# THUDM/GCC

Hardware: AMD Instinct MI355X
Metric: sampled-subgraphs/sec (higher is better)
Workload: dtype f32

## Files before the change

### gcc_amd/csrc/posemb.hip

```cpp
#include <mutex>
#include "host_common.h"
#include <type_traits>

namespace {

constexpr int kJMax = GCC_POSEMB_LDS_MAX;
#ifndef GCC_POSEMB_SMALL_T
#define GCC_POSEMB_SMALL_T 256
#endif
constexpr int kSmallT = GCC_POSEMB_SMALL_T;
constexpr int kJSmall = 64;

constexpr int kMaxViews = GCC_POSEMB_MAX_VIEWS;
struct PosView {
    const int32_t *node_off, *row_ptr, *col_idx;
    float *pos, *evals, *raw;
};
struct PosMulti {
    PosView v[kMaxViews];
    int32_t nviews, B, hidden;
    uint64_t seed;
    int32_t *status;
    long long *ticks;
};
// ... 2090 lines not shown
                }
                __syncthreads();
                orth(j + 1, -1);
                float s3 = 0.f;
                for (int r = tid; r < n; r += kKThreads) s3 = fmaf(w[r], w[r], s3);
                nrm = sqrtf(block_sum(s3, red));
                beta = 0.f;
            } else {
                nrm = beta;
            }
            if (tid == 0) H[(j + 1) * kM + j] = beta;
            for (int r = tid; r < n; r += kKThreads) {
                const float vn = w[r] / nrm;
                V[(int64_t)(j + 1) * ldv + r] = vn;
                x[r] = vn * dinv[r];
            }
            __syncthreads();
        }
        PHASE_TICK(0);
        for (int i = tid; i < kM * lda; i += kKThreads) {
            const int r = i / lda, c = i - r * lda;
            float v = 0.f;
            if (c < kM) v = r <= c ? H[r * kM + c] : H[c * kM + r];
            Aj[i] = v;
        }
        __syncthreads();
        tridiagonalize<1, kKThreads, 2>(Aj, lda, kM, tw);
        eig_top_values<kKThreads, kVecCap>(tw, kM, keep, es);
        const bool ritz_failed = eig_top_vectors<1, kKThreads>(Aj, lda, kM, keep, tw, es,
                                                               (uint32_t)a.seed ^ ((uint32_t)gb * 0x9E3779B1u) ^ (uint32_t)cycle,
                                                               nullptr, tick_);
        PHASE_TICK(1);
        if (tid < kM) {
            theta[tid] = tid < keep ? es.lamv[tid] : -2.f;
            sel[tid] = tid < keep ? tid : kM;
        }
        if (tid == 0) { done = 1; flag = ritz_failed ? 2 : 0; }
        __syncthreads();
        const float beta_m = H[kM * kM + (kM - 1)];
        if (tid < k) {
            const float res = fabsf(beta_m * Yj[(kM - 1) * lda + tid]);
            if (res > kRitzTol) done = 0;
            if (res > 10.f * kRitzTol) flag = 2;
        }
        __syncthreads();
        const bool finished = done != 0 || cycle == kMaxCycles - 1;
#ifdef GCC_AMD_HIPEMU
        if (getenv("GCC_POSEMB_DEBUG") && tid == 0) {
            float worst = 0.f; int nbad = 0;
            for (int i = 0; i < kM; ++i) if (sel[i] < k) { const float rs = fabsf(beta_m * Yj[(kM - 1) * lda + i]); worst = rs > worst ? rs : worst; nbad += rs > kRitzTol; }
            fprintf(stderr, "kry b=%d n=%d cycle=%d worst=%.2e nbad=%d theta_k=%.4f\n", b, n, cycle + 1, worst, nbad, 0.f);
        }
#endif
        if (finished && done == 0 && flag == 2 && tid == 0) {
            atomicOr(a.status, (int32_t)GCC_STATUS_POSEMB_NOT_CONVERGED);
            if (atomicAdd(a.status + 4, 1) == 0) { a.status[5] = gb; a.status[6] = kClsKrylov; a.status[7] = n; a.status[8] = -1; a.status[9] = n; }
        }
        if (finished && done == 0 && tid == 0) atomicAdd(a.status + 3, 1);
        const int nout = finished ? k : keep;
        if (tid < kM) {
            const int t = finished ? k - 1 - sel[tid] : sel[tid];
            if (t >= 0 && t < nout) colsrc[t] = tid;
        }
        __syncthreads();
        if (!finished) {
            const int nchunk = (nout + 7) >> 3;
            for (int task = tid; task < n * nchunk; task += kKThreads) {
                const int ch = task / n, r = task - ch * n;
                float acc[8] = {0.f, 0.f, 0.f, 0.f, 0.f, 0.f, 0.f, 0.f};
                int src[8];
#pragma unroll
                for (int u = 0; u < 8; ++u) src[u] = colsrc[min(8 * ch + u, nout - 1)];
                for (int c = 0; c < kM; ++c) {
                    const float v = V[(int64_t)c * ldv + r];
#pragma unroll
                    for (int u = 0; u < 8; ++u) acc[u] = fmaf(v, Yj[c * lda + src[u]], acc[u]);
                }
#pragma unroll
                for (int u = 0; u < 8; ++u)
                    if (8 * ch + u < nout) Valt[(int64_t)(8 * ch + u) * ldv + r] = acc[u];
            }
            for (int r = tid; r < n; r += kKThreads) Valt[(int64_t)keep * ldv + r] = V[(int64_t)kM * ldv + r];
            for (int i = tid; i < (kM + 1) * kM; i += kKThreads) H[i] = 0.f;
            __syncthreads();
            if (tid < kM && sel[tid] < keep) H[sel[tid] * kM + sel[tid]] = theta[tid];
            __syncthreads();
            float *tmp = V; V = Valt; Valt = tmp;
            j = keep;
            PHASE_TICK(2);
            continue;
        }
        float *rawout = a.raw ? a.raw : a.pos;
        const int nchunk = (k + 7) >> 3;
        for (int task = tid; task < n * nchunk; task += kKThreads) {
            const int ch = task / n, r = task - ch * n;
            float acc[8] = {0.f, 0.f, 0.f, 0.f, 0.f, 0.f, 0.f, 0.f};
            int src[8];
#pragma unroll
            for (int u = 0; u < 8; ++u) src[u] = colsrc[min(8 * ch + u, k - 1)];
            for (int c = 0; c < kM; ++c) {
                const float v = V[(int64_t)c * ldv + r];
#pragma unroll
                for (int u = 0; u < 8; ++u) acc[u] = fmaf(v, Yj[c * lda + src[u]], acc[u]);
            }
            float *ro = rawout + (int64_t)(n0 + r) * a.hidden + 8 * ch;
#pragma unroll
            for (int u = 0; u < 8; ++u)
                if (8 * ch + u < k) ro[u] = acc[u];
        }
        __syncthreads();
        for (int r = tid; r < n; r += kKThreads) {
            const float *ro = rawout + (int64_t)(n0 + r) * a.hidden;
            float *po = a.pos + (int64_t)(n0 + r) * a.hidden;
            float s2 = 0.f;
            for (int c = 0; c < k; ++c) s2 = fmaf(ro[c], ro[c], s2);
            const float inv = s2 > 0.f ? 1.0f / sqrtf(s2) : 1.0f;
            for (int c = 0; c < a.hidden; ++c) {
                const float v = c < k ? ro[c] : 0.f;
                po[c] = v * inv;
                if (a.raw) a.raw[(int64_t)(n0 + r) * a.hidden + c] = v;
            }
        }
        if (a.evals && tid < kM && sel[tid] < k) a.evals[(int64_t)b * a.hidden + (k - 1 - sel[tid])] = theta[tid];
        if (a.evals) for (int c = k + tid; c < a.hidden; c += kKThreads) a.evals[(int64_t)b * a.hidden + c] = 0.f;
        break;
    }
    PHASE_TICK(3);
    if (tid == 0) {
        atomicMax(a.status + 1, cycle + 1);
        atomicAdd(a.status + 2, steps);
    }
    }
}


constexpr int kChP = 64;
constexpr int kChPWide = 64, kChPNarrow = 32;
#ifndef GCC_POSEMB_CH_NARROW_WANT
#define GCC_POSEMB_CH_NARROW_WANT 20
#endif
constexpr int kChNarrowWant = GCC_POSEMB_CH_NARROW_WANT;
constexpr int kChNarrowGuards = 8;
#ifndef GCC_POSEMB_CH_THREADS
#define GCC_POSEMB_CH_THREADS 1024
#endif
constexpr int kChThreads = GCC_POSEMB_CH_THREADS;
static_assert(kChThreads % 64 == 0 && kNodeMax % kChThreads == 0 && kChThreads >= 256 && kChThreads <= 1024, "block-class workgroup size");
constexpr int kChRowsPerThread = kNodeMax / kChThreads;
#if defined(GCC_AMD_HIPEMU) || GCC_POSEMB_CH_THREADS > 512
#define GCC_CHEB_REG_CAP
#else
#define GCC_CHEB_REG_CAP __attribute__((amdgpu_waves_per_eu(GCC_POSEMB_CH_THREADS / 256 + 1)))
#endif
constexpr int kChCsrCap = 12288;
#ifndef GCC_POSEMB_CH_LONGDEG
#define GCC_POSEMB_CH_LONGDEG 32
#endif
constexpr int kChLongDeg = GCC_POSEMB_CH_LONGDEG;
constexpr int kChSlabFloats = 4096;
constexpr int kChMaxChunks = kChSlabFloats / 32;
constexpr int kChMaxLong = kChMaxChunks / 2;
constexpr int kChRounds = 16;
constexpr int kChMaxRitz = 5;
constexpr float kChTol = 2e-5f;
constexpr double kChShift = 1e-8;
constexpr float kChAmpLog = 12.9f;
constexpr int kChBw = 32;

struct LdsYes { static constexpr bool value = true; };
struct LdsNo { static constexpr bool value = false; };

constexpr int64_t kChBufFloats = (int64_t)kNodeMax * kChP;
struct ChebArgs {
    PosMulti m;
    PosHead hd;
    float *xws;
    uint32_t *tabs;
};

template <int P>
struct ChebRitzLds {
    static constexpr int Ldy = P + 1;
    static constexpr int Lf = 0;
    static constexpr int Af = Lf + P * Ldy;
    static constexpr int Y = Af + P * Ldy;
    static constexpr int tri = Y + P * Ldy;
    static constexpr int lu = tri + tri_head_floats(P, P * Ldy, kChThreads);
    static constexpr int bytes = (int)sizeof(float) * lu + tri_lu_bytes(P, kChBw);
};
template <int P>
struct ChebDenseLds {
    static constexpr int G = 0, K = G + P * P, Li = K + P * P;
    static constexpr int bytes = (Li + P * P) * (int)sizeof(double);
};
struct ChebLds {
    static constexpr int crow = 0;
    static constexpr int ccol = crow + (int)sizeof(uint16_t) * (kNodeMax + 8);
    static constexpr int scale = ccol + (int)sizeof(uint16_t) * kChCsrCap;
    static constexpr int slab = scale + (int)sizeof(float) * kNodeMax;
    static constexpr int region = slab + (int)sizeof(float) * kChSlabFloats;
    static constexpr int dense_bytes = ChebDenseLds<kChP>::bytes;
    static constexpr int ritz_pad = kChP * (int)sizeof(float);
    static constexpr int ritz_bytes = ChebRitzLds<kChP>::bytes + ritz_pad;
    static constexpr int region_bytes = ritz_bytes > dense_bytes ? ritz_bytes : dense_bytes;
    static constexpr int bytes = region + region_bytes;
    static_assert(region_bytes >= kNodeMax * kDeflNodeBytes, "the deflation tables overlay the region of the dense matrices");
};

__global__ __launch_bounds__(kChThreads) GCC_CHEB_REG_CAP void posemb_cheb_kernel(ChebArgs ca)
{
    DYN_SMEM(smem);
    __shared__ EigShared es;
    __shared__ float theta[kChP], resid[kChP], dsc[kChP];
    __shared__ double dscd[kChP];
    __shared__ int longrow[kChMaxLong], longfirst[kChMaxLong + 1];
    __shared__ int chunk_beg[kChMaxChunks + 1];
    __shared__ uint8_t chunk_row[kChMaxChunks], rowx[kNodeMax];
    __shared__ int sh_clen, sh_long_t;
    __shared__ int wsum[kChThreads / 64 + 1];
    __shared__ int sh_item, sh_tot[3], sh_nlong, sh_nchunk, sh_fail;
    __shared__ int colsrc[64];
    constexpr int kCls = kClsCheb;
    const PosMulti &m = ca.m;
    const PosHead &hd = ca.hd;
    constexpr int kNW = kChThreads / 64;
    uint16_t *crow = (uint16_t *)(smem + ChebLds::crow);
    uint16_t *ccol = (uint16_t *)(smem + ChebLds::ccol);
    float *scale = (float *)(smem + ChebLds::scale);
    float *slab = (float *)(smem + ChebLds::slab);
    unsigned char *region = smem + ChebLds::region;
    for (;;) {
    __syncthreads();
    if (threadIdx.x == 0) sh_item = atomicAdd(hd.next + kCls, 1);
    __syncthreads();
    if (sh_item >= hd.count[kCls]) return;
    uint32_t tid_ = threadIdx.x;
    opaque_u32(tid_);
    const int tid = (int)tid_, lane = tid & 63, wv = tid >> 6;
    const int gb = hd.list[(int64_t)kCls * hd.T + sh_item] & kItemMask;
    PosArgs a;
    int b;
    item_args(m, gb, a, b);
    const int n0 = a.node_off[b], n = a.node_off[b + 1] - n0;
#ifdef GCC_POSEMB_ABLATE_CHEB
    continue;
#endif
    const int k = min(min(n - 2, a.hidden), kMaxVec);
    long long tick_ = m.ticks ? device_ticks() : 0;
    if (m.ticks && tid == 0) atomicAdd((unsigned long long *)&m.ticks[kCls * 16 + 15], 1ull);
    const int32_t *rp = a.row_ptr + n0;
    float *XA0 = ca.xws + (int64_t)blockIdx.x * 3 * kChBufFloats, *XB0 = XA0 + kChBufFloats, *XC0 = XB0 + kChBufFloats;

    Defl d;
    defl_bind(d, region, kNodeMax);
    for (int i = tid; i < n; i += kChThreads) defl_init_node(d, i, rp, a.col_idx, n0);
    if (tid == 0) { sh_fail = 0; sh_nlong = 0; sh_nchunk = 0; }
    __syncthreads();
    for (int i = tid; i < n; i += kChThreads) defl_count_node(d, i, rp, a.col_idx, n0, hd.use_stalks != 0);
    __syncthreads();
    for (int p = tid; p < n; p += kChThreads) defl_order_node(d, p, rp, a.col_idx, n0);
    __syncthreads();
    defl_prefix_block<kChThreads>(d, n, sh_tot, (int *)slab);
    const int nr = sh_tot[0], z = sh_tot[1], zp = sh_tot[2];
    for (int i = tid; i < n; i += kChThreads) {
        if (d.ridx[i] == kNone) continue;
        const int di = rp[i + 1] - rp[i];
        const int pi = d.par[i];
        float sc = 1.0f / sqrtf((float)(di < 1 ? 1 : di));
        if (pi != (int)kNone && d.tcnt[pi] >= 2) {
            sc = sqrtf((float)d.tcnt[pi]);
        } else {
            const int h = d.phub[pi != (int)kNone ? pi : i];
            if (h != (int)kNone && d.pcnt[h] >= 2) sc = pi != (int)kNone ? 1.0f / sqrtf((float)d.pcnt[h]) : sqrtf(0.5f * (float)d.pcnt[h]);
        }
        scale[d.ridx[i]] = sc;
    }
    for (int r = tid; r <= nr; r += kChThreads) crow[r] = 0;
    __syncthreads();
    for (int i = wv; i < n; i += kNW) {
        if (d.ridx[i] == kNone) continue;
        int c = 0;
        for (int e0 = rp[i]; e0 < rp[i + 1]; e0 += 64) {
            const int e = e0 + lane;
            const bool keep = e < rp[i + 1] && d.ridx[a.col_idx[e] - n0] != kNone;
            c += __popcll(wave_ballot(keep));
        }
        if (lane == 0) crow[d.ridx[i] + 1] = (uint16_t)(c > 65535 ? 65535 : c);
    }
    __syncthreads();
    {
        const int r0 = kChRowsPerThread * tid;
        int c[kChRowsPerThread], own = 0;
#pragma unroll
        for (int u = 0; u < kChRowsPerThread; ++u) { c[u] = r0 + u < nr ? (int)crow[r0 + u + 1] : 0; own += c[u]; }
        int incl = wave_scan_incl(own);
        if (lane == 63) wsum[wv] = incl;
        __syncthreads();
        int base = 0;
        for (int q = 0; q < wv; ++q) base += wsum[q];
        incl += base - own;
        __syncthreads();
#pragma unroll
        for (int u = 0; u < kChRowsPerThread; ++u) {
            incl += c[u];
            if (r0 + u < nr) {
                if (incl > kChCsrCap) sh_fail = 1;
                crow[r0 + u + 1] = (uint16_t)(incl > 65535 ? 65535 : incl);
            }
        }
    }
    __syncthreads();
    if (!sh_fail) {
        for (int i = wv; i < n; i += kNW) {
            if (d.ridx[i] == kNone) continue;
            int at = (int)crow[d.ridx[i]];
            for (int e0 = rp[i]; e0 < rp[i + 1]; e0 += 64) {
                const int e = e0 + lane;
                const int rj = e < rp[i + 1] ? (int)d.ridx[a.col_idx[e] - n0] : (int)kNone;
                const unsigned long long mk = wave_ballot(rj != (int)kNone);
                if (rj != (int)kNone) ccol[at + __popcll(mk & lanemask_lt())] = (uint16_t)rj;
                at += __popcll(mk);
            }
        }
    }
    __syncthreads();
    uint16_t *xrec = (uint16_t *)(ca.tabs + (int64_t)blockIdx.x * kTabFloats);
    for (int v = tid; v < n; v += kChThreads) defl_record(d, v, rp, a.col_idx, n0, xrec + 4 * v);
    __syncthreads();
    PHASE_TICK(0);
    bool failed = sh_fail != 0;
    auto build_chunks = [&](int slots) {
        constexpr int R = kChRowsPerThread;
        const int r0 = R * tid;
        int len[R];
#pragma unroll
        for (int u = 0; u < R; ++u) len[u] = (r0 + u < nr && !failed) ? (int)crow[r0 + u + 1] - (int)crow[r0 + u] : 0;
        auto block_scan = [&](int v, int &total) -> int {
            int incl = wave_scan_incl(v);
            if (lane == 63) wsum[wv] = incl;
            __syncthreads();
            int base = 0, tot = 0;
            for (int q = 0; q < kNW; ++q) { if (q < wv) base += wsum[q]; tot += wsum[q]; }
            __syncthreads();
            total = tot;
            return incl - v + base;
        };
        int T = kChLongDeg, nl = 0, x = 0;
        for (;;) {
            int own = 0;
#pragma unroll
            for (int u = 0; u < R; ++u) own += len[u] > T ? 1 : 0;
            x = block_scan(own, nl);
            if (nl <= slots / 2) break;
            T *= 2;
        }
        int own = 0, total = 0;
#pragma unroll
        for (int u = 0; u < R; ++u) own += len[u] > T ? len[u] : 0;
        (void)block_scan(own, total);
        int clen = nl ? (total + (slots - nl) - 1) / (slots - nl) : 8;
        clen = clen < 8 ? 8 : (clen + 3) & ~3;
        own = 0;
#pragma unroll
        for (int u = 0; u < R; ++u) own += len[u] > T ? (len[u] + clen - 1) / clen : 0;
        int nc = 0;
        int fx = block_scan(own, nc);
#pragma unroll
        for (int u = 0; u < R; ++u) {
            const int r = r0 + u;
            const bool lg = len[u] > T;
            if (r < nr) rowx[r] = lg ? (uint8_t)x : (uint8_t)0xFF;
            if (lg) {
                const int nch = (len[u] + clen - 1) / clen;
                longrow[x] = r;
                longfirst[x] = fx;
                for (int j = 0; j < nch; ++j) { chunk_beg[fx + j] = (int)crow[r] + j * clen; chunk_row[fx + j] = (uint8_t)x; }
                ++x;
                fx += nch;
            }
        }
        if (tid == 0) { longfirst[nl] = nc; sh_nlong = nl; sh_nchunk = nc; sh_clen = clen; sh_long_t = T; }
        __syncthreads();
    };
    const int kq = min(k, nr);
    const bool build_failed = failed;
    auto solve = [&](auto pc) -> int {
    constexpr int P = decltype(pc)::value;
    constexpr int Ldy = P + 1;
    constexpr int E = P * P / kChThreads;
    constexpr int TPM = P / E;
    constexpr int TPR = P / 8;
    constexpr int TPQ = P / 4;
    bool failed = build_failed;
    float *XA = XA0, *XB = XB0, *XC = XC0;
    build_chunks(kChSlabFloats / P);
    const int nchunk = sh_nchunk, nlong = sh_nlong, clen = sh_clen, longT = sh_long_t;
#ifdef GCC_AMD_HIPEMU
    if (getenv("GCC_POSEMB_DEBUG") && tid == 0) fprintf(stderr, "cheb item b=%d n=%d nr=%d nnz=%d nlong=%d nchunk=%d fail=%d P=%d clen=%d T=%d\n", b, n, nr, (int)crow[nr], nlong, nchunk, sh_fail, P, clen, longT);
#endif

    constexpr int kChLdsRows = ChebLds::region_bytes / (P * (int)sizeof(float));
    const bool lds_x = nr <= kChLdsRows;
    auto gather = [&](auto in_lds, const float *src, int e0, int e1, float *acc) {
        const float *base = decltype(in_lds)::value ? (const float *)region : src;
        const int q8 = 8 * (tid % TPR);
        for (int e = e0; e < e1; e += 4) {
            int cj[4];
            float sc[4];
            float4 xa[4], xb[4];
#pragma unroll
            for (int u = 0; u < 4; ++u) {
                const bool in = e + u < e1;
                cj[u] = (int)ccol[in ? e + u : e0];
                sc[u] = in ? scale[cj[u]] : 0.f;
            }
#pragma unroll
            for (int u = 0; u < 4; ++u) {
                xa[u] = *(const float4 *)(base + (int64_t)cj[u] * P + q8);
                xb[u] = *(const float4 *)(base + (int64_t)cj[u] * P + q8 + 4);
            }
#pragma unroll
            for (int u = 0; u < 4; ++u) {
                acc[0] = fmaf(sc[u], xa[u].x, acc[0]); acc[1] = fmaf(sc[u], xa[u].y, acc[1]);
                acc[2] = fmaf(sc[u], xa[u].z, acc[2]); acc[3] = fmaf(sc[u], xa[u].w, acc[3]);
                acc[4] = fmaf(sc[u], xb[u].x, acc[4]); acc[5] = fmaf(sc[u], xb[u].y, acc[5]);
                acc[6] = fmaf(sc[u], xb[u].z, acc[6]); acc[7] = fmaf(sc[u], xb[u].w, acc[7]);
            }
        }
    };
    auto spmm_body = [&](auto in_lds, const float *src, float *dst, float alpha, float center, float gamma) {
        const float *base = decltype(in_lds)::value ? (const float *)region : src;
        uint32_t pt_ = (uint32_t)tid;
        opaque_u32(pt_);
        const int q8 = 8 * ((int)pt_ % TPR), g8 = (int)pt_ / TPR;
        auto finish = [&](int r, const float *acc) {
            const float sr = scale[r];
            const float4 oa = *(const float4 *)(base + (int64_t)r * P + q8), ob = *(const float4 *)(base + (int64_t)r * P + q8 + 4);
            float o[8] = {alpha * (sr * acc[0] - center * oa.x), alpha * (sr * acc[1] - center * oa.y),
                          alpha * (sr * acc[2] - center * oa.z), alpha * (sr * acc[3] - center * oa.w),
                          alpha * (sr * acc[4] - center * ob.x), alpha * (sr * acc[5] - center * ob.y),
                          alpha * (sr * acc[6] - center * ob.z), alpha * (sr * acc[7] - center * ob.w)};
            if (gamma != 0.f) {
                const float4 da = *(const float4 *)(dst + (int64_t)r * P + q8), db = *(const float4 *)(dst + (int64_t)r * P + q8 + 4);
                o[0] -= gamma * da.x; o[1] -= gamma * da.y; o[2] -= gamma * da.z; o[3] -= gamma * da.w;
                o[4] -= gamma * db.x; o[5] -= gamma * db.y; o[6] -= gamma * db.z; o[7] -= gamma * db.w;
            }
            *(float4 *)(dst + (int64_t)r * P + q8) = make_float4(o[0], o[1], o[2], o[3]);
            *(float4 *)(dst + (int64_t)r * P + q8 + 4) = make_float4(o[4], o[5], o[6], o[7]);
        };
        for (int c = g8; c < nchunk; c += kChThreads / TPR) {
            const int r = longrow[chunk_row[c]];
            float acc[8] = {0.f, 0.f, 0.f, 0.f, 0.f, 0.f, 0.f, 0.f};
            gather(in_lds, src, chunk_beg[c], min(chunk_beg[c] + clen, (int)crow[r + 1]), acc);
            *(float4 *)(slab + c * P + q8) = make_float4(acc[0], acc[1], acc[2], acc[3]);
            *(float4 *)(slab + c * P + q8 + 4) = make_float4(acc[4], acc[5], acc[6], acc[7]);
        }
        for (int r = g8; r < nr; r += kChThreads / TPR) {
            const int e0 = (int)crow[r], e1 = (int)crow[r + 1];
            if (e1 - e0 > longT) continue;
            float acc[8] = {0.f, 0.f, 0.f, 0.f, 0.f, 0.f, 0.f, 0.f};
            gather(in_lds, src, e0, e1, acc);
            finish(r, acc);
        }
        if (nchunk) {
            __syncthreads();
            for (int x = g8; x < nlong; x += kChThreads / TPR) {
                float acc[8] = {0.f, 0.f, 0.f, 0.f, 0.f, 0.f, 0.f, 0.f};
// ... 67 lines not shown
        }
        __syncthreads();
#pragma unroll
        for (int ps = 0; ps < kPasses; ++ps) {
            const int r = g8 + ps * RPP;
            if (r < nr) {
                *(float4 *)(xs + r * P + q8) = make_float4(nw[ps][0], nw[ps][1], nw[ps][2], nw[ps][3]);
                *(float4 *)(xs + r * P + q8 + 4) = make_float4(nw[ps][4], nw[ps][5], nw[ps][6], nw[ps][7]);
            }
        }
        __syncthreads();
    };
    auto spmm = [&](const float *src, float *dst, float alpha, float center, float gamma) {
        if (lds_x) {
            float4 *xs = (float4 *)region;
            const float4 *gs = (const float4 *)src;
            for (int i = tid; i < nr * (P / 4); i += kChThreads) xs[i] = gs[i];
            __syncthreads();
            spmm_body(LdsYes(), src, dst, alpha, center, gamma);
        } else {
            spmm_body(LdsNo(), src, dst, alpha, center, gamma);
        }
    };

    using Dense = ChebDenseLds<P>;
    double *G = (double *)region + Dense::G, *K = (double *)region + Dense::K;
    float cut = 0.2f;
    int deg = 6, remaining = 6, round = 0, nrr = 0;
    unsigned long long flops = 0;
    const unsigned long long nnz_ = (unsigned long long)crow[nr], nr_ = (unsigned long long)nr;
    bool converged = false;
    if (!failed) {
        for (int i = tid; i < nr * P; i += kChThreads)
            XA[i] = hash_unit((uint32_t)a.seed ^ ((uint32_t)gb * 0x9E3779B1u), (uint32_t)(i & (P - 1)), (uint32_t)(i / P));
        __syncthreads();
    }
    for (; round < kChRounds && !failed; ++round) {
        uint32_t rt_ = (uint32_t)tid;
        opaque_u32(rt_);
        const int tid = (int)rt_, lane = tid & 63, wv = tid >> 6;
        const int mi = tid / TPM, mj = E * (tid % TPM);
        remaining -= deg;
#ifdef GCC_AMD_HIPEMU
        if (getenv("GCC_POSEMB_RR_ALWAYS")) remaining = 0;
#endif
        const bool rr = remaining <= 0;
        const bool vals_only = rr && nrr == 0, fullrr = rr && !vals_only;
        if (lds_x && !(hd.use_cheb & 4)) {
            const float e = 0.5f * (cut + 1.0f), cen = 0.5f * (cut - 1.0f);
            float sigma = e / (1.0f - cen);
            const float tau = 2.0f / sigma;
            float4 *xs = (float4 *)region;
            for (int i = tid; i < nr * (P / 4); i += kChThreads) xs[i] = ((const float4 *)XA)[i];
            __syncthreads();
            filter_step_lds(XB, sigma / e, cen, 0.f);
            for (int i = 2; i <= deg; ++i) {
                const float sn = 1.0f / (tau - sigma);
                filter_step_lds(XB, 2.0f * sn / e, cen, sigma * sn);
                sigma = sn;
            }
            for (int i = tid; i < nr * (P / 4); i += kChThreads) ((float4 *)XA)[i] = xs[i];
            if (rr) spmm_body(LdsYes(), XA, XB, 1.0f, 0.f, 0.f);
            else __syncthreads();
        } else {
            const float e = 0.5f * (cut + 1.0f), cen = 0.5f * (cut - 1.0f);
            float sigma = e / (1.0f - cen);
            const float tau = 2.0f / sigma;
            spmm(XA, XB, sigma / e, cen, 0.f);
            float *prev = XA, *cur = XB;
            for (int i = 2; i <= deg; ++i) {
                const float sn = 1.0f / (tau - sigma);
                spmm(cur, prev, 2.0f * sn / e, cen, sigma * sn);
                float *t = prev; prev = cur; cur = t;
                sigma = sn;
            }
            if (rr) spmm(XA, XB, 1.0f, 0.f, 0.f);
        }
        flops += (unsigned long long)(deg + (rr ? 1 : 0)) * (2ull * nnz_ * P + 5ull * nr_ * P)
                 + (rr ? 2ull : 1ull) * 2ull * nr_ * P * P + 2ull * P * P * P
                 + (rr ? 4ull * P * P * P : 0ull) + (fullrr ? 2ull : 1ull) * 2ull * nr_ * P * P;
        PHASE_TICK(1);
        {
            constexpr int NB = P / 16;
            constexpr int kUn = 4;
            for (int blk = wv; blk < NB * NB; blk += kNW) {
                const int bi = blk / NB, bj = blk % NB, j = lane & 15, q = lane >> 4;
                const f64x4 z4 = {0.0, 0.0, 0.0, 0.0};
                f64x4 ga[2] = {z4, z4}, ka[2] = {z4, z4};
                const float *xa_ = XA + 16 * bi + j, *xb_ = XA + 16 * bj + j, *wb_ = XB + 16 * bj + j;
                for (int r0 = 0; r0 < nr; r0 += 4 * kUn) {
                    float av[kUn], bv[kUn], wv_[kUn];
#pragma unroll
                    for (int u = 0; u < kUn; ++u) {
                        const int64_t ro = (int64_t)min(r0 + 4 * u + q, nr - 1) * P;
                        av[u] = xa_[ro];
                        bv[u] = xb_[ro];
                        wv_[u] = rr ? wb_[ro] : 0.f;
                    }
#pragma unroll
                    for (int u = 0; u < kUn; ++u) {
                        const bool in = r0 + 4 * u + q < nr;
                        const double a_ = in ? (double)av[u] : 0.0;
                        ga[u & 1] = mfma_16x16x4_f64(a_, (double)bv[u], ga[u & 1]);
                        if (rr) ka[u & 1] = mfma_16x16x4_f64(a_, (double)wv_[u], ka[u & 1]);
                    }
                }
#pragma unroll
                for (int r = 0; r < 4; ++r) {
                    const int row = 16 * bi + q + 4 * r, col = 16 * bj + j;
                    G[row * P + col] = ga[0][r] + ga[1][r];
                    K[row * P + col] = ka[0][r] + ka[1][r];
                }
            }
        }
        __syncthreads();
        PHASE_TICK(5);
        double *Li = (double *)region + Dense::Li;
        if (tid < P) {
            const double dd = G[tid * P + tid];
            const double di = dd > 1e-300 ? 1.0 / sqrt(dd) : 0.0;
            if (!(dd > 1e-300)) sh_fail = 1;
            dsc[tid] = (float)di;
            dscd[tid] = di;
        }
        __syncthreads();
#pragma unroll
        for (int u = 0; u < E; ++u) {
            const int i = mi, j = mj + u;
            const double sc = dscd[i] * dscd[j];
            G[i * P + j] = G[i * P + j] * sc + (i == j ? kChShift : 0.0);
            if (j <= i) {
                const double kv = 0.5 * (K[i * P + j] + K[j * P + i]) * sc;
                Li[i * P + j] = kv;
            }
        }
        __syncthreads();
#pragma unroll
        for (int u = 0; u < E; ++u) {
            const int i = mi, j = mj + u;
            K[i * P + j] = j <= i ? Li[i * P + j] : Li[j * P + i];
        }
        __syncthreads();
        if (wv == 0) {
            double *Lt = Li;
            double ar[32];
            bool bad = false;
            const bool live = lane < P;
#pragma unroll 1
            for (int half = 0; half < P / 32 && !bad; ++half) {
                const int cb = 32 * half;
#pragma unroll
                for (int c = 0; c < 32; ++c) ar[c] = live ? G[lane * P + cb + c] : 0.0;
                if (half == 1) {
#pragma unroll 1
                    for (int k = 0; k < 32; ++k) {
                        const double l = Lt[k * P + lane];
#pragma unroll
                        for (int u = 0; u < 32; ++u) ar[u] = fma(-l, wave_readlane(l, 32 + u), ar[u]);
                    }
                }
                double cap = ar[0];
#pragma unroll 1
                for (int k = cb; k < cb + 32; ++k) {
                    const double piv = wave_readlane(cap, k);
                    if (!(piv > 0.1 * kChShift)) {
#ifdef GCC_AMD_HIPEMU
                        if (getenv("GCC_POSEMB_DEBUG") && lane == 0) fprintf(stderr, "cheb chol fail round=%d col=%d piv=%g\n", round, k, piv);
#endif
                        bad = true;
                        break;
                    }
                    const double l = (live && lane >= k) ? cap * (1.0 / sqrt(piv)) : 0.0;
                    if (live) Lt[k * P + lane] = l;
#pragma unroll
                    for (int jb = 0; jb < 4; ++jb) {
                        if (cb + 8 * jb + 7 > k) {
#pragma unroll
                            for (int u = 0; u < 8; ++u) {
                                const int j = 8 * jb + u;
                                ar[j] = fma(-l, wave_readlane(l, cb + j), ar[j]);
                                if (cb + j == k + 1) cap = ar[j];
                            }
                        }
                    }
                }
            }
            if (bad && lane == 0) sh_fail = 1;
        }
        __syncthreads();
        if (!sh_fail) {
#pragma unroll
            for (int u = 0; u < E; ++u)
                if (mj + u <= mi) G[mi * P + mj + u] = Li[(mj + u) * P + mi];
        }
        __syncthreads();
        if (sh_fail) { failed = true; break; }
        PHASE_TICK(6);
        {
            const int i = mi, j4 = mj;
#pragma unroll
            for (int u = 0; u < E; ++u) {
                const int j = j4 + u;
                Li[i * P + j] = j < i ? G[i * P + j] : (j == i ? 1.0 / G[i * P + i] : 0.0);
            }
            __syncthreads();
            for (int sz = 1; sz < P; sz <<= 1) {
                const int per = sz * sz, pairs = P / (2 * sz);
                for (int e = tid; e < pairs * per; e += kChThreads) {
                    const int pr = e / per, ii = (e - pr * per) / sz, jj = e % sz, r0 = 2 * sz * pr;
                    double acc = 0.0;
                    for (int q = jj; q < sz; ++q) acc += Li[(r0 + sz + ii) * P + r0 + q] * Li[(r0 + q) * P + r0 + jj];
                    Li[(r0 + jj) * P + r0 + sz + ii] = acc;
                }
                __syncthreads();
                for (int e = tid; e < pairs * per; e += kChThreads) {
                    const int pr = e / per, ii = (e - pr * per) / sz, jj = e % sz, r0 = 2 * sz * pr;
                    double acc = 0.0;
                    for (int q = 0; q <= ii; ++q) acc += Li[(r0 + sz + ii) * P + r0 + sz + q] * Li[(r0 + jj) * P + r0 + sz + q];
                    Li[(r0 + sz + ii) * P + r0 + jj] = -acc;
                }
                __syncthreads();
            }
            if (rr) {
                constexpr int NB = P / 16;
                const int jl = lane & 15, ql = lane >> 4;
                const f64x4 z4 = {0.0, 0.0, 0.0, 0.0};
                for (int blk = wv; blk < NB * NB; blk += kNW) {
                    const int bi = blk / NB, bj = blk % NB;
                    f64x4 acc = z4;
                    for (int k0 = 0; k0 < 16 * (bi + 1); k0 += 4) {
                        const int ii = 16 * bi + jl, kk = k0 + ql;
                        const double a_ = kk <= ii ? Li[ii * P + kk] : 0.0;
                        acc = mfma_16x16x4_f64(a_, K[kk * P + 16 * bj + jl], acc);
                    }
#pragma unroll
                    for (int r = 0; r < 4; ++r) G[(16 * bi + ql + 4 * r) * P + 16 * bj + jl] = acc[r];
                }
                __syncthreads();
                for (int blk = wv; blk < NB * NB; blk += kNW) {
                    const int bi = blk / NB, bj = blk % NB;
                    f64x4 acc = z4;
                    for (int k0 = 0; k0 < 16 * (bj + 1); k0 += 4) {
                        const int jj = 16 * bj + jl, kk = k0 + ql;
                        const double b_ = kk <= jj ? Li[jj * P + kk] : 0.0;
                        acc = mfma_16x16x4_f64(G[(16 * bi + jl) * P + kk], b_, acc);
                    }
#pragma unroll
                    for (int r = 0; r < 4; ++r) K[(16 * bi + ql + 4 * r) * P + 16 * bj + jl] = acc[r];
                }
                __syncthreads();
            }
        }
        using Ritz = ChebRitzLds<P>;
        float *Lf = (float *)region + Ritz::Lf, *Af = (float *)region + Ritz::Af;
        {
            float lrow[E], hrow[E];
            const int i = mi, j4 = mj;
#pragma unroll
            for (int u = 0; u < E; ++u) {
                lrow[u] = j4 + u <= i ? (float)Li[i * P + j4 + u] : 0.f;
                hrow[u] = (float)(0.5 * (K[i * P + j4 + u] + K[(j4 + u) * P + i]));
            }
            __syncthreads();
#pragma unroll
            for (int u = 0; u < E; ++u) {
                Lf[i * Ldy + j4 + u] = lrow[u];
                Af[i * Ldy + j4 + u] = hrow[u];
            }
        }
        PHASE_TICK(7);
        TriLds tw;
        tw.Y = (float *)region + Ritz::Y;
        tw.ldy = Ldy;
        tri_bind_head(tw, (float *)region + Ritz::tri, P, P * Ldy);
        tri_bind_lu(tw, (float *)region, Ritz::lu, P, kChBw);
        __syncthreads();
        if (rr) {
            tridiagonalize<1, kChThreads, 2>(Af, Ldy, P, tw);
            eig_top_values<kChThreads, kVecCap>(tw, P, P, es);
            const bool ritz_failed = vals_only ? false
                : eig_top_vectors<1, kChThreads>(Af, Ldy, P, P, tw, es,
                                                 (uint32_t)a.seed ^ ((uint32_t)gb * 0x9E3779B1u) ^ (uint32_t)(round + 77), nullptr, tick_);
#ifdef GCC_AMD_HIPEMU
            if (getenv("GCC_POSEMB_DEBUG") && tid == 0 && ritz_failed) fprintf(stderr, "cheb ritz failed round=%d\n", round);
#endif
            if (ritz_failed) { failed = true; break; }
            ++nrr;
            if (tid < P) theta[tid] = es.lamv[tid];
        }
        PHASE_TICK(2);
        {
            float c[E];
#pragma unroll
            for (int u = 0; u < E; ++u) c[u] = 0.f;
            if (fullrr) {
                for (int q = mi; q < P; ++q) {
                    const float l = Lf[q * Ldy + mi];
#pragma unroll
                    for (int u = 0; u < E; ++u) c[u] = fmaf(l, tw.Y[q * Ldy + mj + u], c[u]);
                }
            } else {
#pragma unroll
                for (int u = 0; u < E; ++u) c[u] = mj + u >= mi ? Lf[(mj + u) * Ldy + mi] : 0.f;
            }
            const float di = dsc[mi];
            __syncthreads();
#pragma unroll
            for (int u = 0; u < E; ++u) Af[mi * P + mj + u] = c[u] * di;
        }
        __syncthreads();
        PHASE_TICK(8);
        {
            constexpr int kRG = kChSlabFloats / P, kG = kChThreads / TPQ, kS = kRG / kG;
            static_assert(kS * kG == kRG, "residual row groups per thread");
            const int q4 = 4 * (tid % TPQ), g16 = tid / TPQ;
            float rs[kS][4];
#pragma unroll
            for (int s = 0; s < kS; ++s) rs[s][0] = rs[s][1] = rs[s][2] = rs[s][3] = 0.f;
            const float t0 = theta[q4], t1 = theta[q4 + 1], t2 = theta[q4 + 2], t3 = theta[q4 + 3];
            for (int r = g16, s = 0; r < nr; r += kG, s = s + 1 == kS ? 0 : s + 1) {
                float xn[4] = {0.f, 0.f, 0.f, 0.f}, wn[4] = {0.f, 0.f, 0.f, 0.f};
                for (int which = 0; which < (fullrr ? 2 : 1); ++which) {
                    const float *src = (which ? XB : XA) + (int64_t)r * P;
                    float o0 = 0.f, o1 = 0.f, o2 = 0.f, o3 = 0.f;
#pragma unroll 1
                    for (int part = 0; part < P / 16; ++part) {
                        float4 rowv[4];
#pragma unroll
                        for (int p = 0; p < 4; ++p) rowv[p] = *(const float4 *)(src + 16 * part + 4 * p);
#pragma unroll
                        for (int p = 0; p < 4; ++p) {
                            const float4 rv = rowv[p];
                            const float xs[4] = {rv.x, rv.y, rv.z, rv.w};
#pragma unroll
                            for (int u = 0; u < 4; ++u) {
                                const float4 cv = *(const float4 *)(Af + (16 * part + 4 * p + u) * P + q4);
                                o0 = fmaf(xs[u], cv.x, o0); o1 = fmaf(xs[u], cv.y, o1);
                                o2 = fmaf(xs[u], cv.z, o2); o3 = fmaf(xs[u], cv.w, o3);
                            }
                        }
                    }
                    if (which) {
                        wn[0] = o0; wn[1] = o1; wn[2] = o2; wn[3] = o3;
                    } else {
                        *(float4 *)(XC + (int64_t)r * P + q4) = make_float4(o0, o1, o2, o3);
                        xn[0] = o0; xn[1] = o1; xn[2] = o2; xn[3] = o3;
                    }
                }
                const float d0 = wn[0] - t0 * xn[0], d1 = wn[1] - t1 * xn[1], d2 = wn[2] - t2 * xn[2], d3 = wn[3] - t3 * xn[3];
#pragma unroll
                for (int u = 0; u < kS; ++u) {
                    if (u != s) continue;
                    rs[u][0] = fmaf(d0, d0, rs[u][0]); rs[u][1] = fmaf(d1, d1, rs[u][1]);
                    rs[u][2] = fmaf(d2, d2, rs[u][2]); rs[u][3] = fmaf(d3, d3, rs[u][3]);
                }
            }
            __syncthreads();
            { float *t = XA; XA = XC; XC = t; }
            if (fullrr) {
#pragma unroll
                for (int u = 0; u < kS; ++u)
                    *(float4 *)(slab + (g16 + u * kG) * P + q4) = make_float4(rs[u][0], rs[u][1], rs[u][2], rs[u][3]);
                __syncthreads();
                if (tid < P) {
                    float sres = 0.f;
                    for (int g = 0; g < kRG; ++g) sres += slab[g * P + tid];
                    resid[tid] = sqrtf(sres);
                }
                __syncthreads();
            }
        }
#ifdef GCC_AMD_HIPEMU
        if (getenv("GCC_POSEMB_DEBUG") && tid == 0) {
            double worst_off = 0, dmin = 1e9, dmax2 = 0, wmax = 0;
            for (int i = 0; i < P; ++i)
                for (int j = 0; j <= i; ++j) {
                    double sdot = 0;
                    for (int r = 0; r < nr; ++r) sdot += (double)XA[(int64_t)r * P + i] * XA[(int64_t)r * P + j];
                    if (i == j) { dmin = sdot < dmin ? sdot : dmin; dmax2 = sdot > dmax2 ? sdot : dmax2; }
                    else worst_off = fabs(sdot) > worst_off ? fabs(sdot) : worst_off;
                }
            for (int i = 0; i < P; ++i) { double sw = 0; for (int r = 0; r < nr; ++r) sw += (double)XB[(int64_t)r * P + i] * XB[(int64_t)r * P + i]; wmax = sw > wmax ? sw : wmax; }
            fprintf(stderr, "cheb gram-after-rotate round=%d rr=%d P=%d deg=%d: diag [%g, %g] offdiag %g  max|W col|^2 %g\n", round, (int)rr, P, deg, dmin, dmax2, worst_off, wmax);
        }
        __syncthreads();
#endif
        PHASE_TICK(3);
        if (rr) {
            int kw = kq;
            if (zp > 0) {
                int nge = 0;
                for (int j = 0; j < kq; ++j) if (theta[j] >= kStalkEig - 1e-3f) nge = j + 1;
                kw = max(max(nge, min(kq, k - zp)), 1);
            }
            if (P < kChPWide && kw > P - kChNarrowGuards) return 2;
            float worst = 0.1f;
            if (fullrr) {
                worst = 0.f;
                for (int i = 0; i < kw; ++i) worst = fmaxf(worst, resid[i]);
            }
#ifdef GCC_AMD_HIPEMU
            if (getenv("GCC_POSEMB_DEBUG") && tid == 0)
                fprintf(stderr, "cheb b=%d n=%d nr=%d zp=%d round=%d deg=%d cut=%.4f worst=%.2e kw=%d theta[kw-1]=%.5f theta[P-1]=%.5f\n", b, n, nr, zp, round,
                        deg, cut, worst, kw, theta[kw - 1], theta[P - 1]);
#endif
            if (fullrr && worst <= kChTol) { converged = true; ++round; break; }
            if (nrr >= kChMaxRitz) break;
            cut = fminf(fmaxf(theta[P - 1] - 0.02f, -0.9f), 0.9f);
            const float e = 0.5f * (cut + 1.0f), cen = 0.5f * (cut - 1.0f);
            const float xk = fmaxf((theta[kw - 1] - cen) / e, 1.0001f);
            const float rate = logf(xk + sqrtf(xk * xk - 1.0f));
            int need = (int)(2.3f * logf(fmaxf(worst, 1e-3f) / (0.5f * kChTol)) / rate) + 4;
            remaining = need < 4 ? 4 : (need > 60 ? 60 : need);
        }
        {
            const float x1 = (1.0f - 0.5f * (cut - 1.0f)) / (0.5f * (cut + 1.0f));
            const float ach = logf(x1 + sqrtf(x1 * x1 - 1.0f));
            int dmax = (int)(kChAmpLog / ach) & ~1;
            dmax = dmax < 4 ? 4 : (dmax > 24 ? 24 : dmax);
            deg = ((remaining + 1) & ~1) < dmax ? ((remaining + 1) & ~1) : dmax;
            if (deg < 2) deg = 2;
        }
    }
    if (converged) {
        __syncthreads();
        if (tid == 0) {
            const int na = rank_columns(theta, kq, k, z, zp, colsrc, nullptr);
            bool ok = na == 0 || theta[na - 1] > 10.f * kZeroEig;
            for (int t = 0; t < k; ++t) {
                const int src = colsrc[t];
                if (src < 0 && (src > -kStalkSrc || ((-src - kStalkSrc) & 1))) ok = false;
            }
            sh_fail = ok ? 0 : 1;
        }
        __syncthreads();
        if (sh_fail) converged = false;
    }
    if (!converged) {
        if (tid == 0) {
            int cls = nr <= kGMax ? kClsSlot : (nr <= kBMax ? kClsBig : kClsKrylov);
            if (n > kNodeMax) cls = kClsKrylov;
            if (cls == kClsKrylov && n >= hd.ldv) {
                atomicOr(a.status, (int32_t)GCC_STATUS_POSEMB_TOO_LARGE);
                cls = -1;
            }
            if (cls >= 0) hd.list[(int64_t)cls * hd.T + atomicAdd(hd.count + cls, 1)] = gb | kItemCopies;
            atomicAdd(a.status + 3, 1);
            sh_fail = cls < 0 ? 2 : 1;
        }
        __syncthreads();
        if (sh_fail == 2) {
            for (int i = tid; i < n * a.hidden; i += kChThreads) a.pos[(int64_t)n0 * a.hidden + i] = 0.f;
            if (a.evals) for (int i = tid; i < a.hidden; i += kChThreads) a.evals[(int64_t)b * a.hidden + i] = 0.f;
        }
        return 0;
    }
    if (a.evals) {
        for (int i = tid; i < a.hidden; i += kChThreads)
            a.evals[(int64_t)b * a.hidden + i] = i < k ? (colsrc[i] >= 0 ? theta[colsrc[i]] : kStalkEig) : 0.f;
    }
    for (int v = wv; v < n; v += kNW) {
        const int rsrc = xrec[4 * v], o = xrec[4 * v + 1], g = xrec[4 * v + 2], cb = xrec[4 * v + 3];
        const float val = lane < k ? defl_expand(rsrc, o, g, cb, colsrc[lane], XA, P) : 0.f;
        const float s2 = wave_sum(val * val);
        const float inv = s2 > 0.f ? 1.0f / sqrtf(s2) : 1.0f;
        if (lane < a.hidden) {
            a.pos[(int64_t)(n0 + v) * a.hidden + lane] = val * inv;
            if (a.raw) a.raw[(int64_t)(n0 + v) * a.hidden + lane] = val;
        }
    }
    PHASE_TICK(4);
    if (m.ticks && tid == 0) atomicAdd((unsigned long long *)&m.ticks[kCls * 16 + 14], flops);
    if (tid == 0) atomicMax(a.status + 1, round);
    return 0;
    };
    const int want = max(min(kq, k - zp), 1);
    int rc = 2;
    if (!(hd.use_cheb & 2) && want <= kChNarrowWant) rc = solve(std::integral_constant<int, kChPNarrow>());
    if (rc == 2) {
        __syncthreads();
        solve(std::integral_constant<int, kChPWide>());
    }
    }
}

}

extern "C" {

static long long *g_posemb_ticks = nullptr;
struct PosGrids { int32_t small, mid, slot, kry, big, cheb, w48, w64, pair; };

struct PosKnobs {
    int caps[9];
    int gcaps[2];
    bool sort;
    int use_cheb;
    bool use_wave;
    bool use_stalks;
    bool use_pair;
    int fork;
};
static PosKnobs posemb_knobs(void)
{
    static const PosKnobs once = [] {
        PosKnobs k = {{256, 64, 128, 64, 64, 96, 128, 64, 192}, {128, 128}, true, 1, true, true, true, 0};
        int *c = k.caps, *g = k.gcaps;
        if (const char *e = getenv("GCC_POSEMB_GRID_CAPS"))
            (void)sscanf(e, "%d,%d,%d,%d,%d,%d,%d,%d,%d", &c[0], &c[1], &c[2], &c[3], &c[4], &c[5], &c[6], &c[7], &c[8]);
        if (const char *e = getenv("GCC_POSEMB_GATED_CAPS")) (void)sscanf(e, "%d,%d", &g[0], &g[1]);
        for (int i = 0; i < 9; ++i) c[i] = c[i] < 1 ? 1 : c[i];
        for (int i = 0; i < 2; ++i) g[i] = g[i] < 1 ? 1 : g[i];
        if (const char *e = getenv("GCC_POSEMB_SORT")) k.sort = atoi(e) != 0;
        return k;
    }();
    PosKnobs k = once;
    if (const char *e = getenv("GCC_POSEMB_CHEB")) k.use_cheb = atoi(e);
    if (const char *e = getenv("GCC_POSEMB_WAVE")) k.use_wave = atoi(e) != 0;
    if (const char *e = getenv("GCC_POSEMB_STALKS")) k.use_stalks = atoi(e) != 0;
    if (const char *e = getenv("GCC_POSEMB_PAIR")) k.use_pair = atoi(e) != 0;
    if (const char *e = getenv("GCC_POSEMB_FORK")) k.fork = atoi(e);
    return k;
}

static PosGrids posemb_grids(const PosKnobs &k, int64_t T, bool gated)
{
    const int *caps = k.caps;
    auto lim = [](int64_t want, int cap) { return (int32_t)(want < cap ? want : cap); };
    PosGrids g;
    g.small = lim(T, caps[0]);
    g.mid = lim((T + 3) / 4, gated ? k.gcaps[0] : caps[1]);
    g.slot = lim((T + 7) / 8, caps[2]);
    g.kry = lim((T + 15) / 16, caps[3]);
    g.big = lim((T + 15) / 16, caps[4]);
    g.cheb = lim((T + 7) / 8, gated ? k.gcaps[1] : caps[5]);
    const int64_t wg = (T + kWaveTeams - 1) / kWaveTeams;
    g.w48 = lim(wg, caps[6]);
    g.w64 = lim((wg + 1) / 2, caps[7]);
    g.pair = lim((T + 1) / 2, gated ? 2 * caps[8] : caps[8]);
    return g;
}
static PosGrids posemb_grids_for_sizing(const PosKnobs &k, int64_t T)
{
    PosGrids a = posemb_grids(k, T, false);
    const PosGrids b = posemb_grids(k, T, true);
    a.mid = a.mid > b.mid ? a.mid : b.mid;
    a.cheb = a.cheb > b.cheb ? a.cheb : b.cheb;
    a.pair = a.pair > b.pair ? a.pair : b.pair;
    return a;
}
static int64_t posemb_ldv(int32_t batch_size, int64_t node_cap) { return ((node_cap / batch_size + 63) / 64) * 64 + 64; }

struct PosWorkLayout {
    PosGrids gs;
    int64_t ldv;
    int64_t head;
    int64_t slots;
    int64_t bslots;
    int64_t tabs;
    int64_t vws;
    int64_t xws;
    int64_t ctabs;
    int64_t pslots;
    int64_t total;
};
constexpr int64_t kWorkKeptPad = 768;
static PosWorkLayout posemb_work_layout(const PosKnobs &k, int32_t num_views, int32_t batch_size, int64_t node_cap)
{
    const int64_t T = (int64_t)num_views * batch_size, F = (int64_t)sizeof(float);
    PosWorkLayout l;
    l.gs = posemb_grids_for_sizing(k, T);
    l.ldv = posemb_ldv(batch_size, node_cap);
    int64_t at = 0;
    auto take = [&at](int64_t bytes) { const int64_t off = at; at = (at + bytes + 255) / 256 * 256; return off; };
    l.head = take((16 + kNumCls * T) * 4);
    l.slots = take(l.gs.slot * DirectSlot<kGMax>::floats * F);
    l.bslots = take(l.gs.big * DirectSlot<kBMax>::floats * F);
    l.tabs = take((int64_t)(l.gs.mid + l.gs.small) * kTabFloats * F);
    l.vws = take(l.gs.kry * kry_basis_floats(l.ldv) * F);
    l.xws = take(l.gs.cheb * 3 * kChBufFloats * F);
    l.ctabs = take((int64_t)l.gs.cheb * kTabFloats * F);
    (void)take(kWorkKeptPad);
    l.pslots = take((int64_t)l.gs.pair * PairSlot::floats * F);
    l.total = at;
    return l;
}

static int g_posemb_fork = -1;
#ifndef GCC_AMD_HIPEMU
struct PosSide { hipStream_t owner, side[2]; hipEvent_t fork, join[2]; };
static PosSide *posemb_side_streams(hipStream_t s)
{
    static std::mutex mu;
    static PosSide tab[16];
    static int ntab = 0;
    std::lock_guard<std::mutex> lk(mu);
    for (int i = 0; i < ntab; ++i)
        if (tab[i].owner == s) return &tab[i];
    if (ntab == 16) return nullptr;
    PosSide &t = tab[ntab];
    int prio = 0;
    if (hipStreamGetPriority(s, &prio) != hipSuccess) { (void)hipGetLastError(); prio = 0; }
    for (int i = 0; i < 2; ++i) {
        if (hipStreamCreateWithPriority(&t.side[i], hipStreamNonBlocking, prio) != hipSuccess) { (void)hipGetLastError(); return nullptr; }
        if (hipEventCreateWithFlags(&t.join[i], hipEventDisableTiming) != hipSuccess) { (void)hipGetLastError(); return nullptr; }
    }
    if (hipEventCreateWithFlags(&t.fork, hipEventDisableTiming) != hipSuccess) { (void)hipGetLastError(); return nullptr; }
    t.owner = s;
    return &tab[ntab++];
}
#endif

int64_t gcc_posemb_multi_workspace_bytes(int32_t num_views, int32_t batch_size, int64_t node_cap, int32_t hidden)
{
    if (num_views < 1 || num_views > kMaxViews || batch_size < 1 || node_cap < 1 || hidden < 2 || hidden > kMaxVec) {
        snprintf(g_err, kErrLen, "gcc_posemb_multi_workspace_bytes: bad argument");
        return -1;
    }
    return posemb_work_layout(posemb_knobs(), num_views, batch_size, node_cap).total;
}

// ... 159 lines not shown
```

Before: 716,700.

## Split long-row ordering, group CSR build lanes, pipeline Cholesky pivots, pack output waves

Several independent changes to the Chebyshev posemb kernel. Node ordering for high-degree hub rows now runs one wave per row with ballots, and the compact CSR build uses small lane groups per row, with a wave-per-row fallback only for rows longer than 64. The blocked Cholesky prefetches the next Lt row and computes the next pivot ahead of the trailing update to shorten the dependency chain. The output stage packs two nodes per wave with half-wave DPP reductions and keeps four nodes in flight. These add register pressure and code complexity, and the hidden size is assumed to be at most 32 in the output path.

```diff
diff --git a/gcc_amd/csrc/posemb.hip b/gcc_amd/csrc/posemb.hip
--- a/gcc_amd/csrc/posemb.hip
+++ b/gcc_amd/csrc/posemb.hip
@@ -2266,6 +2266,11 @@
 #else
 #define GCC_CHEB_REG_CAP __attribute__((amdgpu_waves_per_eu(GCC_POSEMB_CH_THREADS / 256 + 1)))
 #endif
+constexpr int kChGrp = kChThreads / 128 < 4 ? 4 : kChThreads / 128;
+constexpr int kChGrpRows = kChThreads / kChGrp;
+constexpr int kChGrpPasses = kNodeMax / kChGrpRows;
+static_assert((kChGrp & (kChGrp - 1)) == 0 && 64 % kChGrp == 0 && kNodeMax % kChGrpRows == 0, "lane groups of the matrix build");
+constexpr int kChOrderWave = 16;
 constexpr int kChCsrCap = 12288;
 #ifndef GCC_POSEMB_CH_LONGDEG
 #define GCC_POSEMB_CH_LONGDEG 32
@@ -2280,6 +2285,23 @@
 constexpr double kChShift = 1e-8;
 constexpr float kChAmpLog = 12.9f;
 constexpr int kChBw = 32;
+
+__device__ __forceinline__ float half32_tree_sum(float v)
+{
+#ifdef GCC_AMD_HIPEMU
+    for (int d = 16; d >= 1; d >>= 1) v += wave_shfl_xor(v, d);
+    return v;
+#else
+    v += dpp_or_zero<0x111, 0xF>(v);
+    v += dpp_or_zero<0x112, 0xF>(v);
+    v += dpp_or_zero<0x114, 0xF>(v);
+    v += dpp_or_zero<0x118, 0xF>(v);
+    v += dpp_or_zero<0x142, 0xA>(v);
+    const float t31 = __int_as_float(__builtin_amdgcn_readlane(__float_as_int(v), 31));
+    const float t63 = __int_as_float(__builtin_amdgcn_readlane(__float_as_int(v), 63));
+    return lane_id() < 32 ? t31 : t63;
+#endif
+}
 
 struct LdsYes { static constexpr bool value = true; };
 struct LdsNo { static constexpr bool value = false; };
@@ -2332,7 +2354,7 @@
     __shared__ uint8_t chunk_row[kChMaxChunks], rowx[kNodeMax];
     __shared__ int sh_clen, sh_long_t;
     __shared__ int wsum[kChThreads / 64 + 1];
-    __shared__ int sh_item, sh_tot[3], sh_nlong, sh_nchunk, sh_fail;
+    __shared__ int sh_item, sh_tot[3], sh_nlong, sh_nchunk, sh_fail, sh_nlongrow;
     __shared__ int colsrc[64];
     constexpr int kCls = kClsCheb;
     const PosMulti &m = ca.m;
@@ -2368,12 +2390,42 @@
     Defl d;
     defl_bind(d, region, kNodeMax);
     for (int i = tid; i < n; i += kChThreads) defl_init_node(d, i, rp, a.col_idx, n0);
-    if (tid == 0) { sh_fail = 0; sh_nlong = 0; sh_nchunk = 0; }
+    if (tid == 0) { sh_fail = 0; sh_nlong = 0; sh_nchunk = 0; sh_nlongrow = 0; }
     __syncthreads();
     for (int i = tid; i < n; i += kChThreads) defl_count_node(d, i, rp, a.col_idx, n0, hd.use_stalks != 0);
     __syncthreads();
-    for (int p = tid; p < n; p += kChThreads) defl_order_node(d, p, rp, a.col_idx, n0);
-    __syncthreads();
+    uint16_t *longlist = (uint16_t *)slab;
+    for (int p = tid; p < n; p += kChThreads) {
+        if (rp[p + 1] - rp[p] > kChOrderWave && (d.tcnt[p] >= 2 || d.pcnt[p] >= 2)) longlist[atomicAdd(&sh_nlongrow, 1)] = (uint16_t)p;
+        else defl_order_node(d, p, rp, a.col_idx, n0);
+    }
+    __syncthreads();
+    for (int x = wv, nx = sh_nlongrow; x < nx; x += kNW) {
+        const int p = longlist[x];
+        const bool lt = d.tcnt[p] >= 2, st = d.pcnt[p] >= 2;
+        int o = 0, q = 0;
+        for (int e0 = rp[p]; e0 < rp[p + 1]; e0 += 64) {
+            const bool in = e0 + lane < rp[p + 1];
+            const int j = in ? a.col_idx[e0 + lane] - n0 : 0;
+            const bool tw = in && lt && d.par[j] == (uint16_t)p;
+            const bool sk = in && !tw && st && d.phub[j] == (uint16_t)p;
+            const unsigned long long mt = wave_ballot(tw), ms = wave_ballot(sk);
+            if (tw) {
+                const int r = o + __popcll(mt & lanemask_lt());
+                if (r == 0) d.rep[p] = (uint16_t)j;
+                d.ord[j] = (uint16_t)r;
+            }
+            if (sk) {
+                const int r = q + __popcll(ms & lanemask_lt());
+                if (r == 0) d.prep[p] = (uint16_t)j;
+                d.ord[j] = (uint16_t)r;
+            }
+            o += __popcll(mt);
+            q += __popcll(ms);
+        }
+    }
+    __syncthreads();
+    if (tid == 0) sh_nlongrow = 0;
     defl_prefix_block<kChThreads>(d, n, sh_tot, (int *)slab);
     const int nr = sh_tot[0], z = sh_tot[1], zp = sh_tot[2];
     for (int i = tid; i < n; i += kChThreads) {
@@ -2391,8 +2443,37 @@
     }
     for (int r = tid; r <= nr; r += kChThreads) crow[r] = 0;
     __syncthreads();
-    for (int i = wv; i < n; i += kNW) {
-        if (d.ridx[i] == kNone) continue;
+    const int gl = lane & (kChGrp - 1), grp = tid / kChGrp;
+    const unsigned long long gmask = ((1ull << kChGrp) - 1ull) << (lane - gl);
+    int g_e0[kChGrpPasses], g_len[kChGrpPasses], g_ri[kChGrpPasses], g_rj[kChGrpPasses];
+#pragma unroll
+    for (int p = 0; p < kChGrpPasses; ++p) {
+        const int i = p * kChGrpRows + grp;
+        g_ri[p] = i < n ? (int)d.ridx[i] : (int)kNone;
+        g_e0[p] = i < n ? rp[i] : 0;
+        g_len[p] = g_ri[p] != (int)kNone ? rp[i + 1] - g_e0[p] : 0;
+        if (g_len[p] > 64) {
+            if (gl == 0) longlist[atomicAdd(&sh_nlongrow, 1)] = (uint16_t)i;
+            g_len[p] = 0;
+        }
+    }
+#pragma unroll
+    for (int p = 0; p < kChGrpPasses; ++p)
+        g_rj[p] = gl < g_len[p] ? (int)d.ridx[a.col_idx[g_e0[p] + gl] - n0] : (int)kNone;
+#pragma unroll
+    for (int p = 0; p < kChGrpPasses; ++p) {
+        if (p * kChGrpRows >= n) break;
+        int c = __popcll(wave_ballot(g_rj[p] != (int)kNone) & gmask);
+        for (int r = kChGrp; wave_ballot(r < g_len[p]) != 0ull; r += kChGrp) {
+            const bool keep = r + gl < g_len[p] && d.ridx[a.col_idx[g_e0[p] + r + gl] - n0] != kNone;
+            c += __popcll(wave_ballot(keep) & gmask);
+        }
+        if (gl == 0 && g_ri[p] != (int)kNone && g_len[p] > 0) crow[g_ri[p] + 1] = (uint16_t)c;
+    }
+    __syncthreads();
+    const int nlongrow = sh_nlongrow;
+    for (int x = wv; x < nlongrow; x += kNW) {
+        const int i = longlist[x];
         int c = 0;
         for (int e0 = rp[i]; e0 < rp[i + 1]; e0 += 64) {
             const int e = e0 + lane;
@@ -2425,8 +2506,22 @@
     }
     __syncthreads();
     if (!sh_fail) {
-        for (int i = wv; i < n; i += kNW) {
-            if (d.ridx[i] == kNone) continue;
+#pragma unroll
+        for (int p = 0; p < kChGrpPasses; ++p) {
+            if (p * kChGrpRows >= n) break;
+            int at = g_len[p] > 0 ? (int)crow[g_ri[p]] : 0;
+            unsigned long long mk = wave_ballot(g_rj[p] != (int)kNone) & gmask;
+            if (g_rj[p] != (int)kNone) ccol[at + __popcll(mk & lanemask_lt())] = (uint16_t)g_rj[p];
+            at += __popcll(mk);
+            for (int r = kChGrp; wave_ballot(r < g_len[p]) != 0ull; r += kChGrp) {
+                const int rj = r + gl < g_len[p] ? (int)d.ridx[a.col_idx[g_e0[p] + r + gl] - n0] : (int)kNone;
+                mk = wave_ballot(rj != (int)kNone) & gmask;
+                if (rj != (int)kNone) ccol[at + __popcll(mk & lanemask_lt())] = (uint16_t)rj;
+                at += __popcll(mk);
+            }
+        }
+        for (int x = wv; x < nlongrow; x += kNW) {
+            const int i = longlist[x];
             int at = (int)crow[d.ridx[i]];
             for (int e0 = rp[i]; e0 < rp[i + 1]; e0 += 64) {
                 const int e = e0 + lane;
@@ -2800,37 +2895,54 @@
 #pragma unroll
                 for (int c = 0; c < 32; ++c) ar[c] = live ? G[lane * P + cb + c] : 0.0;
                 if (half == 1) {
+                    double ln = Lt[lane];
 #pragma unroll 1
                     for (int k = 0; k < 32; ++k) {
-                        const double l = Lt[k * P + lane];
+                        const double l = ln;
+                        ln = Lt[(k < 31 ? k + 1 : 31) * P + lane];
 #pragma unroll
                         for (int u = 0; u < 32; ++u) ar[u] = fma(-l, wave_readlane(l, 32 + u), ar[u]);
                     }
                 }
-                double cap = ar[0];
+                double piv = wave_readlane(ar[0], cb);
+                bool ok = piv > 0.1 * kChShift;
+                double l = (live && lane >= cb) ? ar[0] * (1.0 / sqrt(piv)) : 0.0;
 #pragma unroll 1
                 for (int k = cb; k < cb + 32; ++k) {
-                    const double piv = wave_readlane(cap, k);
-                    if (!(piv > 0.1 * kChShift)) {
+                    if (!ok) {
 #ifdef GCC_AMD_HIPEMU
                         if (getenv("GCC_POSEMB_DEBUG") && lane == 0) fprintf(stderr, "cheb chol fail round=%d col=%d piv=%g\n", round, k, piv);
 #endif
                         bad = true;
                         break;
                     }
-                    const double l = (live && lane >= k) ? cap * (1.0 / sqrt(piv)) : 0.0;
                     if (live) Lt[k * P + lane] = l;
+                    const int kn = k + 1 - cb;
+                    double nx = 0.0;
 #pragma unroll
                     for (int jb = 0; jb < 4; ++jb) {
-                        if (cb + 8 * jb + 7 > k) {
-#pragma unroll
-                            for (int u = 0; u < 8; ++u) {
-                                const int j = 8 * jb + u;
-                                ar[j] = fma(-l, wave_readlane(l, cb + j), ar[j]);
-                                if (cb + j == k + 1) cap = ar[j];
-                            }
+                        if ((kn >> 3) == jb) {
+#pragma unroll
+                            for (int t = 0; t < 8; ++t)
+                                if ((kn & 7) == t) nx = ar[8 * jb + t];
                         }
                     }
+                    nx = fma(-l, wave_readlane(l, (k + 1) & 63), nx);
+                    piv = wave_readlane(nx, (k + 1) & 63);
+                    ok = piv > 0.1 * kChShift;
+                    const double lnx = nx * (1.0 / sqrt(piv));
+                    keep_alive(lnx);
+                    const double ln = (live && lane > k) ? lnx : 0.0;
+#pragma unroll
+                    for (int j = 24; j < 32; ++j) ar[j] = fma(-l, wave_readlane(l, cb + j), ar[j]);
+#pragma unroll
+                    for (int jb = 0; jb < 3; ++jb) {
+                        if (cb + 8 * jb + 7 > k) {
+#pragma unroll
+                            for (int u = 0; u < 8; ++u) ar[8 * jb + u] = fma(-l, wave_readlane(l, cb + 8 * jb + u), ar[8 * jb + u]);
+                        }
+                    }
+                    l = ln;
                 }
             }
             if (bad && lane == 0) sh_fail = 1;
@@ -3107,14 +3219,28 @@
         for (int i = tid; i < a.hidden; i += kChThreads)
             a.evals[(int64_t)b * a.hidden + i] = i < k ? (colsrc[i] >= 0 ? theta[colsrc[i]] : kStalkEig) : 0.f;
     }
-    for (int v = wv; v < n; v += kNW) {
-        const int rsrc = xrec[4 * v], o = xrec[4 * v + 1], g = xrec[4 * v + 2], cb = xrec[4 * v + 3];
-        const float val = lane < k ? defl_expand(rsrc, o, g, cb, colsrc[lane], XA, P) : 0.f;
-        const float s2 = wave_sum(val * val);
-        const float inv = s2 > 0.f ? 1.0f / sqrtf(s2) : 1.0f;
-        if (lane < a.hidden) {
-            a.pos[(int64_t)(n0 + v) * a.hidden + lane] = val * inv;
-            if (a.raw) a.raw[(int64_t)(n0 + v) * a.hidden + lane] = val;
+    {
+        const int hl = lane & 31, hv = lane >> 5;
+        const int src = hl < k ? colsrc[hl] : 0;
+        auto node_value = [&](int v) -> float {
+            if (v >= n || hl >= k) return 0.f;
+            const int rsrc = xrec[4 * v], o = xrec[4 * v + 1], g = xrec[4 * v + 2], cb = xrec[4 * v + 3];
+            return defl_expand(rsrc, o, g, cb, src, XA, P);
+        };
+        auto node_store = [&](int v, float val, float s2) {
+            const float inv = s2 > 0.f ? 1.0f / sqrtf(s2) : 1.0f;
+            if (v < n && hl < a.hidden) {
+                a.pos[(int64_t)(n0 + v) * a.hidden + hl] = val * inv;
+                if (a.raw) a.raw[(int64_t)(n0 + v) * a.hidden + hl] = val;
+            }
+        };
+        constexpr int kFly = 4;
+        for (int v0 = 2 * wv; v0 < n; v0 += 2 * kFly * kNW) {
+            float x[kFly];
+#pragma unroll
+            for (int f = 0; f < kFly; ++f) x[f] = node_value(v0 + hv + 2 * kNW * f);
+#pragma unroll
+            for (int f = 0; f < kFly; ++f) node_store(v0 + hv + 2 * kNW * f, x[f], half32_tree_sum(x[f] * x[f]));
         }
     }
     PHASE_TICK(4);
```

Measured after the change: 726,400, median of 6. 1.01x the previous value.
